# CLSFramework/gym-soccer-2d-env

Measured on AMD Instinct MI355X. Metric: env-steps/sec at 65536 parallel reach_ball envs per MI355X, higher is better.
Workload: dtype f32

## Files before the change

gym-soccer-2d-env_amd/csrc/s2d_engine.hip:

```cpp
#include <hip/hip_runtime.h>

#include <cmath>
#include <cstdio>
#include <cstdlib>
#include <cstring>
#include <new>
#include <string>
#include <type_traits>

#include "s2d_device.h"

#include "s2d_kernels.h"

__global__ void s2d_tables_kernel(S2DHot p, const S2DRare* __restrict__ rp, S2DTables* __restrict__ t) {
  if (blockIdx.x == 0 && threadIdx.x == 0 && rp->tab_len > 0) tables_build(p, rp->recover_init, rp->tab_power, rp->tab_len, *t);
}
__global__ __launch_bounds__(kBlock) void s2d_init_kernel(S2DHot p, const S2DRare* __restrict__ rp,
                                                          float* __restrict__ S, int64_t stride, int64_t n) {
  int64_t i = (int64_t)blockIdx.x * kBlock + threadIdx.x;
  if (i >= n) return;
  S[F_STAMINA * stride + i] = p.stamina_max;
  S[F_RECOVERY * stride + i] = rp->recover_init;
  S[F_EFFORT * stride + i] = p.effort_init;
  S[F_CAPACITY * stride + i] = p.stamina_capacity;
// ... 341 lines not shown
    if (p.auto_reset) n_missing += __popcll(__ballot(active && done != 0));
    if (ro.obs) store_obs_tile(lds[wv], ob, lane, active, ro.obs + (row + wave_first) * S2D_OBS_DIM, valid);
  }
  if (active) {
    if (fast) {
      const int q = e.step_number;
      e.stamina = tb->stamina[q]; e.effort = tb->effort[q]; e.recovery = tb->recovery[q]; e.capacity = tb->capacity[q];
    }
    env_store(e, S, stride, i);
    if (use_k) kplane[i] = k0 + (uint32_t)n_steps;
    o.reward[i] = reward; o.done[i] = (uint8_t)done; o.result[i] = (uint8_t)res;
    o.action_dir[i] = dir; o.action_cmd[i] = (uint8_t)cmd;
  }
  store_obs_tile(lds[wv], ob, lane, active, o.obs + wave_first * S2D_OBS_DIM, valid);
  if (!active) { cnt1 = cnt2 = cnt3 = 0; }
#pragma unroll
  for (int off = 32; off > 0; off >>= 1) {
    cnt1 += __shfl_xor(cnt1, off); cnt2 += __shfl_xor(cnt2, off); cnt3 += __shfl_xor(cnt3, off);
  }
  unsigned long long* const srow = stats_row(o.stats, wave_first);
  stats_store(srow, lane, stats_load(srow, lane), wave_first == 0 ? (unsigned long long)n * (unsigned long long)n_steps : 0ull, cnt1, cnt2, cnt3);
}

#ifndef S2D_NPRIO_S
#define S2D_NPRIO_S 3
#endif
#ifndef S2D_NPRIO_A
#define S2D_NPRIO_A 2
#endif
#ifndef S2D_NPRIO_B
#define S2D_NPRIO_B 2
#endif
#ifndef S2D_NPRIO_P
#define S2D_NPRIO_P 1
#endif
#ifndef S2D_PRIO_S
#define S2D_PRIO_S 1
#endif
#ifndef S2D_PRIO_A
#define S2D_PRIO_A 2
#endif
#ifndef S2D_PRIO_B
#define S2D_PRIO_B 3
#endif

#ifdef S2D_STAMPS
#define WS_STAMP_DECL uint64_t st_busy = 0, st_t0 = __builtin_amdgcn_s_memtime(); const uint64_t st_begin = st_t0, st_rt0 = __builtin_amdgcn_s_memrealtime()
#define WS_BARRIER() do { st_busy += __builtin_amdgcn_s_memtime() - st_t0; __syncthreads(); st_t0 = __builtin_amdgcn_s_memtime(); } while (0)
#define WS_STAMP_STORE() do { if (lane == 0) { float* q_ = o.terminal_obs + (wave_first + 2 * role) * S2D_OBS_DIM; \
    q_[0] = (float)st_busy; q_[1] = (float)(__builtin_amdgcn_s_memtime() - st_begin); q_[2] = (float)(st_rt0 & 0xffffff); \
    q_[3] = (float)(__builtin_amdgcn_s_memrealtime() & 0xffffff); \
    q_[4] = __int_as_float((int)__builtin_amdgcn_s_getreg((31 << 11) | 4)); q_[5] = __int_as_float((int)__builtin_amdgcn_s_getreg((31 << 11) | 20)); } } while (0)
#else
#define WS_STAMP_DECL do {} while (0)
#define WS_BARRIER() __syncthreads()
#define WS_STAMP_STORE() do {} while (0)
#endif

template <int MODE, int NK, int REC = 0>
__global__ __launch_bounds__(kWsBlock, 4) void s2d_reach_rollout_ws_kernel(S2DHot p_sgpr, const S2DRare* __restrict__ rp,
                                                                        float* __restrict__ S, int64_t stride,
                                                                        int64_t n, int n_steps,
                                                                        const void* __restrict__ actions, int kind,
                                                                        RolloutOut ro, StepOut o) {
  constexpr bool NOISE = NK != S2D_NK_OFF;
  constexpr int kActWords = NOISE ? (int)WA_WORDS : (int)WA_NPM;
  __shared__ float act[3][kActWords][kWave];
  __shared__ float snap[2][WS_WORDS][kWave];
  __shared__ float slots[kSlots][SL_WORDS][kWave];
  __shared__ __attribute__((aligned(16))) float tile[2][kObsTile];
  __shared__ float4 act_lut[kWave];
  __shared__ float ep_lds[S2D_TAB_MAX];
  __shared__ float2 sc_lut[361];
  const int lane = threadIdx.x & (kWave - 1);
  const int role = __builtin_amdgcn_readfirstlane(threadIdx.x / kWave);
  const bool nt = REC == 2 || (REC == 0 && ro.nt != 0);
  const int64_t wave_first = (int64_t)blockIdx.x * kWave;
  const int64_t i = wave_first + lane;
  const bool active = i < n;
  int64_t rows = n - wave_first; rows = rows > kWave ? kWave : rows;
  const int valid = (int)rows * S2D_OBS_DIM;
  const int n_iter = n_steps + 3;

  if (role != 1 && p_sgpr.auto_reset) {
    const uint64_t gid = (((uint64_t)p_sgpr.gid_hi << 32) | p_sgpr.gid_lo) + (uint64_t)i;
    uint32_t ep0 = 0u;
    if (active) ep0 = reinterpret_cast<const uint32_t*>(S + F_EPISODE * stride)[i];
    const int k = role == 0 ? 0 : role - 1;
    slot_fill_coop<NK>(p_sgpr, rp, slots[k], lane, (uint32_t)gid, (uint32_t)(gid >> 32), ep0 + 1u + (uint32_t)k, active,
                          reinterpret_cast<uint32_t*>(&tile[0][0]) + role * kWave);
  }

  if (role == 0) {
    if constexpr (NOISE) __builtin_amdgcn_s_setprio(S2D_NPRIO_P);
    const S2DHot& p = p_sgpr;
    const bool use_k = uses_policy_step<MODE, NOISE>(kind);
    uint32_t* const kplane = reinterpret_cast<uint32_t*>(S + F_POLICY * stride);
    uint32_t gl = 0, gh = 0, k0 = 0;
    if (active) {
      if (use_k) k0 = kplane[i];
      uint64_t gid = (((uint64_t)p.gid_hi << 32) | p.gid_lo) + (uint64_t)i;
      gl = (uint32_t)gid; gh = (uint32_t)(gid >> 32);
    }
    U4 quad{0, 0, 0, 0}, squad{0, 0, 0, 0}, nblk{0, 0, 0, 0};
    float dir = 0.0f; int cmd = 0;
    int64_t row = 0;
    const bool lut = MODE == S2D_MODE_DISCRETE && kind == S2D_ACT_RANDOM && p.n_actions <= kWave;
    if (lut && lane < p.n_actions) {
      int c0; float pw, d0;
      action_map<MODE>(p, Action4{(float)lane, 0.0f, 0.0f, 0.0f}, 0.0f, c0, pw, d0);
      const CmdPrep c = cmd_prepare(p, c0, pw, d0);
      act_lut[lane] = make_float4(c.power, c.dir, c.dir_rate, d0);
    }
    __syncthreads();
    WS_STAMP_DECL;
    int wslot = 0;
    auto policy_step = [&](int t) {
      if (active) {
        const uint32_t k = k0 + (uint32_t)t;
        CmdPrep c;
        if (lut) {
          if (t == 0 || (k & 3u) == 0u) quad = policy_quad(p, gl, gh, k, S2D_ST_POLICY);
          const int a = (int)rnd_below(quad_word(quad, k), (uint32_t)p.n_actions);
          if (REC != 0 || ro.action) rec_store(static_cast<int32_t*>(ro.action) + row + i, (int32_t)a, nt);
          const float4 e4 = act_lut[a];
          c = CmdPrep{e4.x, e4.y, e4.z}; dir = e4.w; cmd = S2D_CMD_DASH;
        } else {
          c = decide<MODE>(p, actions, kind, row + i, gl, gh, k, t == 0 || (k & 3u) == 0u, quad, squad, ro.action, cmd, dir);
        }
        const int b = wslot;
        if (MODE == S2D_MODE_TURN4) act[b][WA_CMD][lane] = __int_as_float(cmd);
        act[b][WA_POWER][lane] = c.power;
        act[b][WA_DIR][lane] = c.dir; act[b][WA_RATE][lane] = c.dir_rate;
        if constexpr (NK == S2D_NK_SQUARE) {
          const NoiseIn nz = noise_prepare_square(p, gl, gh, k, S2D_ST_NOISE, cmd == S2D_CMD_TURN);
          act[b][WA_NPM][lane] = nz.pm; act[b][WA_NPS][lane] = nz.ps; act[b][WA_NPC][lane] = nz.pc;
          act[b][WA_NBM][lane] = nz.bm; act[b][WA_NBS][lane] = nz.bs; act[b][WA_NBC][lane] = nz.bc;
          if (MODE == S2D_MODE_TURN4) act[b][WA_NTU][lane] = nz.tu;
        } else if constexpr (NOISE) {
          const NoiseWords nw = noise_words(p, gl, gh, k, S2D_ST_NOISE, cmd == S2D_CMD_TURN, nblk, t == 0 || (k & 1u) == 0u);
          const float2 ps = sc_lut[noise_dir_index(nw.wp)], bs = sc_lut[noise_dir_index(nw.wb)];
          act[b][WA_NPM][lane] = noise_mag(nw.wp); act[b][WA_NPS][lane] = ps.x; act[b][WA_NPC][lane] = ps.y;
          act[b][WA_NBM][lane] = noise_mag(nw.wb); act[b][WA_NBS][lane] = bs.x; act[b][WA_NBC][lane] = bs.y;
          if (MODE == S2D_MODE_TURN4) act[b][WA_NTU][lane] = nw.tu;
        }
        row += n;
      }
      wslot = wslot == 2 ? 0 : wslot + 1;
    };
    for (int s = 0; s < n_iter; ++s) {
      if (s == 0 && n_steps > 0) policy_step(0);
      if (s + 1 < n_steps) policy_step(s + 1);
      WS_BARRIER();
    }
    WS_STAMP_STORE();
    if (active) {
      if (use_k) kplane[i] = k0 + (uint32_t)n_steps;
      o.action_dir[i] = dir; o.action_cmd[i] = (uint8_t)cmd;
    }
  } else if (role == 1) {
    if constexpr (NOISE) __builtin_amdgcn_s_setprio(S2D_NPRIO_S);
    else __builtin_amdgcn_s_setprio(S2D_PRIO_S);
    const S2DHot p = hot_in_vgprs(p_sgpr);
    Env e;
    uint32_t gl = 0, gh = 0;
    int nth = 0, j = 0;
    if (active) {
      env_load(e, S, stride, i);
      uint64_t gid = (((uint64_t)p.gid_hi << 32) | p.gid_lo) + (uint64_t)i;
      gl = (uint32_t)gid; gh = (uint32_t)(gid >> 32);
      asm volatile("" ::"v"(e.px), "v"(e.py), "v"(e.vx), "v"(e.vy), "v"(e.body), "v"(e.stamina), "v"(e.effort),
                   "v"(e.recovery), "v"(e.capacity), "v"(e.bx), "v"(e.by), "v"(e.bvx), "v"(e.bvy),
                   "v"(e.step_number), "v"(e.cycle), "v"(e.episode));
    }
    const S2DTables* const tb = tables_of(rp);
    const int tab_len = MODE != S2D_MODE_TURN4 ? rp->tab_len : 0;
    bool fast = false;
    if (tab_len > 0) {
      bool ok = true;
      if (active) {
        const int sn = e.step_number;
        ok = sn >= 0 && sn < tab_len;
        const int q = ok ? sn : 0;
        ok = ok && e.stamina == tb->stamina[q] && e.effort == tb->effort[q] && e.recovery == tb->recovery[q] &&
             e.capacity == tb->capacity[q] && e.body == rintf(e.body) && fabsf(e.body) <= 180.0f;
      }
      fast = __ballot(active && !ok) == 0ull;
      if (fast)
        for (int k = lane; k < tab_len; k += kWave) ep_lds[k] = tb->ep[k];
    }
    if (fast || NK == S2D_NK_LATTICE) {
      for (int k = lane; k <= 360; k += kWave) {
        float sn, cs;
        sincos_deg((float)(k - 180), sn, cs);
        sc_lut[k] = make_float2(sn, cs);
      }
    }
    const ResetStamina rst = reset_stamina(p, rp);
    __syncthreads();
    WS_STAMP_DECL;
    auto loop = [&](auto fast_tag) {
      constexpr bool FAST = decltype(fast_tag)::value;
      struct ActRegs { float cmd, power, dir, rate, npm, nps, npc, nbm, nbs, nbc, ntu; };
      ActRegs cur{}, nxt{};
      float ep_cur = 0.0f; float2 sc_cur = make_float2(0.0f, 0.0f);
      int rslot = 1;
      auto fetch = [&](int slot) {
        ActRegs r{};
        if (MODE == S2D_MODE_TURN4) r.cmd = act[slot][WA_CMD][lane];
        if (!FAST) r.power = act[slot][WA_POWER][lane];
        r.dir = act[slot][WA_DIR][lane]; r.rate = act[slot][WA_RATE][lane];
        if constexpr (NOISE) {
          r.npm = act[slot][WA_NPM][lane]; r.nps = act[slot][WA_NPS][lane]; r.npc = act[slot][WA_NPC][lane];
          r.nbm = act[slot][WA_NBM][lane]; r.nbs = act[slot][WA_NBS][lane]; r.nbc = act[slot][WA_NBC][lane];
          if (MODE == S2D_MODE_TURN4) r.ntu = act[slot][WA_NTU][lane];
        }
        return r;
      };
      auto lookups = [&]() {
        if constexpr (FAST) {
          ep_cur = ep_lds[e.step_number];
          sc_cur = sc_lut[(int)norm_deg(e.body + cur.dir) + 180];
        }
      };
      auto simulate_iteration = [&](int s, auto steady_tag) {
        constexpr bool STEADY = decltype(steady_tag)::value;
        if ((STEADY || (s >= 1 && s <= n_steps)) && active) {
          if (!STEADY && s == 1) { cur = fetch(0); lookups(); }
          const bool more = STEADY || s < n_steps;
          if (more) nxt = fetch(rslot);
          const int b = (s - 1) & 1;
          int cmd = S2D_CMD_DASH;
          if (MODE == S2D_MODE_TURN4) cmd = __float_as_int(cur.cmd);
          NoiseIn nz{0.0f, 0.0f, 0.0f, 0.0f, 0.0f, 0.0f, 0.0f};
          if constexpr (NOISE) {
            nz = NoiseIn{cur.npm, cur.nps, cur.npc, cur.nbm, cur.nbs, cur.nbc, 0.0f};
            if (MODE == S2D_MODE_TURN4) nz.tu = cur.ntu;
          }
          float d2;
          if constexpr (FAST) {
            e.step_number += 1;
            d2 = sim_cycle_dash_fast<NOISE>(p, rp, e, ep_cur, cur.rate, sc_cur.x, sc_cur.y, nz);
          } else {
            const CmdPrep c{cur.power, cur.dir, cur.rate};
            e.step_number += 1;
            d2 = sim_cycle<NOISE, true>(p, rp, e, cmd, c, nz);
          }
          int flags = judge_sq(p, e.px, e.py, d2, e.step_number);
          const bool took = flags && p.auto_reset;
          snap[b][WS_PX][lane] = e.px; snap[b][WS_PY][lane] = e.py; snap[b][WS_BODY][lane] = e.body;
          snap[b][WS_BX][lane] = e.bx; snap[b][WS_BY][lane] = e.by;
          snap[b][WS_BVX][lane] = e.bvx; snap[b][WS_BVY][lane] = e.bvy;
          snap[b][WS_FLAGS][lane] = __int_as_float(flags | (j << 8));
          if (took) {
            if (nth >= kSlots)
              slot_fill<NK>(p, rp, slots[j], lane, gl, gh, (uint32_t)e.episode + 1u);
            episode_begin(e, slot_take<kWave>(slots[j], lane, rst));
            nth += 1; j = (j + 1 == kSlots) ? 0 : j + 1;
          }
          if (more) { cur = nxt; lookups(); }
        }
        if (STEADY || (s >= 1 && s < n_steps)) rslot = rslot == 2 ? 0 : rslot + 1;
        WS_BARRIER();
      };
      int s = 0;
      for (; s < 2 && s < n_iter; ++s) simulate_iteration(s, std::false_type{});
      for (; s < n_steps; ++s) simulate_iteration(s, std::true_type{});
      for (; s < n_iter; ++s) simulate_iteration(s, std::false_type{});
    };
    if (fast) {
      loop(std::true_type{});
      if (active) {
        const int q = e.step_number;
        e.stamina = tb->stamina[q]; e.effort = tb->effort[q]; e.recovery = tb->recovery[q]; e.capacity = tb->capacity[q];
      }
    } else {
      loop(std::false_type{});
    }
    WS_STAMP_STORE();
    if (active) {
      S[F_PX * stride + i] = e.px; S[F_PY * stride + i] = e.py;
      S[F_VX * stride + i] = e.vx; S[F_VY * stride + i] = e.vy;
      S[F_BODY * stride + i] = e.body;
      S[F_STAMINA * stride + i] = e.stamina; S[F_EFFORT * stride + i] = e.effort;
      S[F_RECOVERY * stride + i] = e.recovery; S[F_CAPACITY * stride + i] = e.capacity;
      S[F_BX * stride + i] = e.bx; S[F_BY * stride + i] = e.by;
      S[F_BVX * stride + i] = e.bvx; S[F_BVY * stride + i] = e.bvy;
      S[F_STEP * stride + i] = __int_as_float(e.step_number);
      S[F_CYCLE * stride + i] = __int_as_float(e.cycle);
      S[F_EPISODE * stride + i] = __int_as_float(e.episode);
    }
  } else if (role == 2) {
    __builtin_amdgcn_s_setprio(NOISE ? S2D_NPRIO_A : S2D_PRIO_A);
    const S2DHot p = hot_in_vgprs(p_sgpr);
    const bool auto_reset = p_sgpr.auto_reset != 0;
    float prev_dist = 0.0f, prev_angle = 0.0f;
    if (active) {
      prev_dist = S[F_PREV_DIST * stride + i]; prev_angle = S[F_PREV_ANGLE * stride + i];
      asm volatile("" ::"v"(prev_dist), "v"(prev_angle));
    }
    float oa[S2D_OBS_DIM];
    float reward = 0.0f; int res = 0, done = 0;
    unsigned int cnt1 = 0, cnt2 = 0, cnt3 = 0;
    unsigned long long* const srow = stats_row(o.stats, wave_first);
    const unsigned long long sold = stats_load(srow, lane);
    float* const term_row = o.terminal_obs + i * S2D_OBS_DIM;
    int64_t row = 0;
    __syncthreads();
    WS_STAMP_DECL;
    auto agent_iteration = [&](int s, auto steady_tag) {
      constexpr bool STEADY = decltype(steady_tag)::value;
      if (STEADY || (s >= 2 && s < n_steps + 2)) {
        const int b = s & 1;
        res = 0;
        if (active) {
          float px = snap[b][WS_PX][lane], py = snap[b][WS_PY][lane], body = snap[b][WS_BODY][lane];
          float bx = snap[b][WS_BX][lane], by = snap[b][WS_BY][lane];
          const int fw = __float_as_int(snap[b][WS_FLAGS][lane]);
          const int flags = fw & 0xff;
          float dist = hypot2(bx - px, by - py);
          float rel = observe_player(p, px, py, body, bx, by, oa);
          reward = reward_of(prev_dist, prev_angle, dist, rel, flags, res);
          prev_dist = dist; prev_angle = rel;
          done = flags ? 1 : 0;
          if (flags && auto_reset) {
            const float (*sl)[kWave] = slots[fw >> 8];
#pragma unroll
            for (int k = 0; k < 4; ++k) term_row[k] = oa[k];
#pragma unroll
            for (int k = 0; k < 4; ++k) oa[k] = sl[SL_FIRST + k][lane];
            prev_dist = sl[SL_DIST][lane]; prev_angle = sl[SL_REL][lane];
          }
          if (REC != 0 || ro.reward) rec_store(ro.reward + row + i, reward, nt);
          if (REC != 0 || ro.done) rec_store(ro.done + row + i, (uint8_t)done, nt);
          if (REC != 0 || ro.result) rec_store(ro.result + row + i, (uint8_t)res, nt);
          cnt1 += res == S2D_RESULT_GOAL; cnt2 += res == S2D_RESULT_OUT; cnt3 += res == S2D_RESULT_TIMEOUT;
          if (REC != 0 || ro.obs) {
            float* t = &tile[b][lane * S2D_OBS_DIM];
            t[0] = oa[0]; t[1] = oa[1]; t[2] = oa[2]; t[3] = oa[3];
          }
        }
        row += n;
      }
      WS_BARRIER();
    };
    {
      int s = 0;
      for (; s < 3 && s < n_iter; ++s) agent_iteration(s, std::false_type{});
      for (; s < n_steps + 2; ++s) agent_iteration(s, std::true_type{});
      for (; s < n_iter; ++s) agent_iteration(s, std::false_type{});
    }
    WS_STAMP_STORE();
    if (active) {
      S[F_PREV_DIST * stride + i] = prev_dist; S[F_PREV_ANGLE * stride + i] = prev_angle;
      o.reward[i] = reward; o.done[i] = (uint8_t)done; o.result[i] = (uint8_t)res;
#pragma unroll
      for (int k = 0; k < 4; ++k) o.obs[i * S2D_OBS_DIM + k] = oa[k];
    }
    if (!active) { cnt1 = cnt2 = cnt3 = 0; }
#pragma unroll
    for (int off = 32; off > 0; off >>= 1) {
      cnt1 += __shfl_xor(cnt1, off); cnt2 += __shfl_xor(cnt2, off); cnt3 += __shfl_xor(cnt3, off);
    }
    stats_store(srow, lane, sold, wave_first == 0 ? (unsigned long long)n * (unsigned long long)n_steps : 0ull, cnt1, cnt2, cnt3);
  } else {
    if constexpr (NOISE) __builtin_amdgcn_s_setprio(S2D_NPRIO_B);
    else __builtin_amdgcn_s_setprio(S2D_PRIO_B);
    const S2DHot p = hot_in_vgprs(p_sgpr);
    const bool auto_reset = p_sgpr.auto_reset != 0;
    float ob6[S2D_OBS_DIM];
    float* const term_row = o.terminal_obs + i * S2D_OBS_DIM;
    const bool obs_all_vec = valid == kObsTile && ((n * S2D_OBS_DIM * 4) & 15) == 0 &&
                             (reinterpret_cast<uintptr_t>(ro.obs + wave_first * S2D_OBS_DIM) & 15u) == 0;
    __syncthreads();
    WS_STAMP_DECL;
    auto ball_iteration = [&](int s, auto steady_tag) {
      constexpr bool STEADY = decltype(steady_tag)::value;
      if ((STEADY || s >= 3) && (REC != 0 || ro.obs))
        tile_flush(tile[(s - 1) & 1], lane, ro.obs + ((int64_t)(s - 3) * n + wave_first) * S2D_OBS_DIM, valid, nt, obs_all_vec);
      if ((STEADY || (s >= 2 && s < n_steps + 2)) && active) {
        const int b = s & 1;
        float bx = snap[b][WS_BX][lane], by = snap[b][WS_BY][lane];
        float bvx = snap[b][WS_BVX][lane], bvy = snap[b][WS_BVY][lane];
        const int fw = __float_as_int(snap[b][WS_FLAGS][lane]);
        observe_ball(p, bx, by, bvx, bvy, ob6);
        if ((fw & 0xff) && auto_reset) {
          const float (*sl)[kWave] = slots[fw >> 8];
#pragma unroll
          for (int k = 4; k < S2D_OBS_DIM; ++k) term_row[k] = ob6[k];
#pragma unroll
          for (int k = 4; k < S2D_OBS_DIM; ++k) ob6[k] = sl[SL_FIRST + k][lane];
        }
        if (REC != 0 || ro.obs) {
          float* t = &tile[b][lane * S2D_OBS_DIM];
#pragma unroll
          for (int k = 4; k < S2D_OBS_DIM; ++k) t[k] = ob6[k];
        }
      }
      WS_BARRIER();
    };
    {
      int s = 0;
      for (; s < 3 && s < n_iter; ++s) ball_iteration(s, std::false_type{});
      for (; s < n_steps + 2; ++s) ball_iteration(s, std::true_type{});
      for (; s < n_iter; ++s) ball_iteration(s, std::false_type{});
    }
    WS_STAMP_STORE();
    if (active) {
#pragma unroll
      for (int k = 4; k < S2D_OBS_DIM; ++k) o.obs[i * S2D_OBS_DIM + k] = ob6[k];
    }
  }
}

__global__ __launch_bounds__(kBlock) void s2d_world_model_kernel(const float* __restrict__ S, int64_t stride,
                                                                 int64_t n, S2DWorldModel w) {
  int64_t i = (int64_t)blockIdx.x * kBlock + threadIdx.x;
  if (i >= n) return;
  float px = S[F_PX * stride + i], py = S[F_PY * stride + i], vx = S[F_VX * stride + i], vy = S[F_VY * stride + i];
  float bx = S[F_BX * stride + i], by = S[F_BY * stride + i], bvx = S[F_BVX * stride + i], bvy = S[F_BVY * stride + i];
  float dx = bx - px, dy = by - py;
  float dist = hypot2(dx, dy), ang = atan2_deg(dy, dx);
  if (w.ball_dist_from_self) w.ball_dist_from_self[i] = dist;
  if (w.ball_angle_from_self) w.ball_angle_from_self[i] = ang;
  if (w.ball_relative_x) w.ball_relative_x[i] = dx;
  if (w.ball_relative_y) w.ball_relative_y[i] = dy;
  if (w.ball_pos_dist) w.ball_pos_dist[i] = hypot2(bx, by);
  if (w.ball_pos_angle) w.ball_pos_angle[i] = atan2_deg(by, bx);
  if (w.ball_vel_dist) w.ball_vel_dist[i] = hypot2(bvx, bvy);
  if (w.ball_vel_angle) w.ball_vel_angle[i] = atan2_deg(bvy, bvx);
  if (w.self_pos_dist) w.self_pos_dist[i] = hypot2(px, py);
  if (w.self_pos_angle) w.self_pos_angle[i] = atan2_deg(py, px);
  if (w.self_vel_dist) w.self_vel_dist[i] = hypot2(vx, vy);
  if (w.self_vel_angle) w.self_vel_angle[i] = atan2_deg(vy, vx);
  if (w.self_dist_from_ball) w.self_dist_from_ball[i] = dist;
  if (w.self_angle_from_ball) w.self_angle_from_ball[i] = atan2_deg(-dy, -dx);
}

enum { SV_NONFINITE, SV_BODY, SV_STAMINA, SV_EFFORT_RECOVERY, SV_COUNTERS, SV_OBS, SV_WORDS = 8 };
__global__ __launch_bounds__(kBlock) void s2d_validate_kernel(S2DHot p, const float* __restrict__ S, int64_t stride, int64_t n,
                                                              const float* __restrict__ obs, unsigned int* __restrict__ out) {
  const int64_t i = (int64_t)blockIdx.x * kBlock + threadIdx.x;
  if (i >= n) return;
  Env e;
  env_load(e, S, stride, i);
  const float w[15] = {e.px, e.py, e.vx, e.vy, e.body, e.stamina, e.effort, e.recovery, e.capacity, e.bx, e.by, e.bvx, e.bvy,
                       e.prev_dist, e.prev_angle};
  bool finite = true;
#pragma unroll
  for (int k = 0; k < 15; ++k) finite = finite && isfinite(w[k]);
  bool obs_ok = true;
#pragma unroll
  for (int k = 0; k < S2D_OBS_DIM; ++k) obs_ok = obs_ok && isfinite(obs[i * S2D_OBS_DIM + k]);
  if (!finite) atomicAdd(&out[SV_NONFINITE], 1u);
  if (!(fabsf(e.body) <= 180.0f) || !(fabsf(e.prev_angle) <= 180.0f)) atomicAdd(&out[SV_BODY], 1u);
  if (!(e.stamina >= 0.0f && e.stamina <= p.stamina_max) || !(e.capacity >= 0.0f || p.stamina_capacity < 0.0f)) atomicAdd(&out[SV_STAMINA], 1u);
  if (!(e.effort >= p.effort_min && e.effort <= p.effort_init) || !(e.recovery >= p.recover_min && e.recovery <= p.recover_init))
    atomicAdd(&out[SV_EFFORT_RECOVERY], 1u);
  if (e.step_number < 0 || e.episode < 0 || !(e.prev_dist >= 0.0f)) atomicAdd(&out[SV_COUNTERS], 1u);
  if (!obs_ok) atomicAdd(&out[SV_OBS], 1u);
}

__global__ void s2d_debug_eval_kernel(int op, const float* __restrict__ in, float* __restrict__ out, int64_t n) {
  int64_t i = (int64_t)blockIdx.x * blockDim.x + threadIdx.x;
  if (op == 9) {
    __shared__ uint32_t scratch[256];
    const uint32_t* u = reinterpret_cast<const uint32_t*>(in) + 4 * i;
    S2DHot p{}; p.seed_lo = u[2]; p.seed_hi = 0x5EEDu; p.half_l = 52.5f; p.half_w = 34.0f;
    S2DRare r{}; r.change_ball_position = 1; r.change_ball_velocity = 1; r.travel_factor = __uint_as_float(u[3]);
    const int lane = threadIdx.x & 63;
    const ResetSample a = reset_sample_coop(p, r, (uint32_t)i, 7u, u[0], u[1] != 0u, lane, scratch + (threadIdx.x & ~63u));
    const ResetSample b = reset_sample(p, r, (uint32_t)i, 7u, u[0]);
    float* q = out + 14 * i;
    q[0] = a.px; q[1] = a.py; q[2] = a.body; q[3] = a.bx; q[4] = a.by; q[5] = a.bvx; q[6] = a.bvy;
    q[7] = b.px; q[8] = b.py; q[9] = b.body; q[10] = b.bx; q[11] = b.by; q[12] = b.bvx; q[13] = b.bvy;
    return;
  }
  if (i >= n) return;
  switch (op) {
    case 10: {
      const uint32_t* u = reinterpret_cast<const uint32_t*>(in) + 4 * i;
      S2DHot p{}; p.seed_lo = u[3]; p.seed_hi = 0u;
      const NoiseIn nz = noise_prepare(p, u[0], u[1], u[2], S2D_ST_NOISE, false);
      float* q = out + 6 * i;
      q[0] = nz.pm; q[1] = nz.ps; q[2] = nz.pc; q[3] = nz.bm; q[4] = nz.bs; q[5] = nz.bc;
      break;
    }
    case 11:
    case 12: {
// ... 663 lines not shown
```

gym-soccer-2d-env_amd/csrc/s2d_kernels.h:

```cpp
#pragma once
#include <hip/hip_runtime.h>

#include <type_traits>

#include "s2d_device.h"
#include "s2d_net.h"

#define S2D_API extern "C" __attribute__((visibility("default")))

#ifndef S2D_BLOCK
#define S2D_BLOCK 256
#endif
static constexpr int kBlock = S2D_BLOCK;
static constexpr int kWavesPerBlock = kBlock / kWave;
static constexpr int kObsTile = kWave * S2D_OBS_DIM;
static constexpr int64_t kWsMaxEnvs = 524288;

struct StepOut {
  float* obs;
  float* reward;
  uint8_t* done;
  uint8_t* result;
  float* terminal_obs;
  float* action_dir;
  uint8_t* action_cmd;
  unsigned long long* stats;
  float* prep;
};

enum { PS_PX, PS_PY, PS_BODY, PS_BX, PS_BY, PS_BVX, PS_BVY, PS_WORDS };
S2D_DEV uint32_t* prep_tags(float* prep, int64_t stride) { return reinterpret_cast<uint32_t*>(prep + 2 * PS_WORDS * stride); }
static constexpr uint32_t kPrepTagMask = 0x3fffffffu;
S2D_DEV uint32_t prep_tag_of(uint32_t episode, const NextEpisode& q) {
  return (episode & kPrepTagMask) | ((uint32_t)__float_as_int(q.vx) & 0x80000000u) | (((uint32_t)__float_as_int(q.vy) & 0x80000000u) >> 1);
}

S2D_DEV void wave_lds_fence() {
  __builtin_amdgcn_fence(__ATOMIC_RELEASE, "wavefront");
  __builtin_amdgcn_wave_barrier();
  __builtin_amdgcn_fence(__ATOMIC_ACQUIRE, "wavefront");
}

S2D_DEV void tile_write(float* tile, const ObsOut& ob, int lane, bool active) {
  if (active) {
#pragma unroll
    for (int k = 0; k < S2D_OBS_DIM; ++k) tile[lane * S2D_OBS_DIM + k] = ob.o[k];
  }
}
typedef float v4f32_t __attribute__((ext_vector_type(4)));
S2D_DEV void rec_store16(float4* p, const float4& v, bool nt) {
  if (nt) {
    const v4f32_t w = {v.x, v.y, v.z, v.w};
    asm volatile("global_store_dwordx4 %0, %1, off nt" ::"v"(p), "v"(w) : "memory");
  } else {
    *p = v;
  }
}
template <typename T>
S2D_DEV void rec_store(T* p, T v, bool nt) {
  if (nt) __builtin_nontemporal_store(v, p); else *p = v;
}
S2D_DEV void tile_flush(const float* tile, int lane, float* __restrict__ dst, int valid, bool nt = false, bool all_vec = false) {
  const bool vec = all_vec || ((valid == kObsTile) && ((reinterpret_cast<uintptr_t>(dst) & 15u) == 0));
  if (vec) {
    const float4* t4 = reinterpret_cast<const float4*>(tile);
    float4* d4 = reinterpret_cast<float4*>(dst);
    rec_store16(d4 + lane, t4[lane], nt);
    rec_store16(d4 + kWave + lane, t4[kWave + lane], nt);
    if (lane < 32) rec_store16(d4 + 2 * kWave + lane, t4[2 * kWave + lane], nt);
  } else {
#pragma unroll
    for (int j = 0; j < S2D_OBS_DIM; ++j) {
      int idx = j * kWave + lane;
      if (idx < valid) dst[idx] = tile[idx];
    }
  }
}
S2D_DEV void store_obs_tile(float* tile, const ObsOut& ob, int lane, bool active, float* __restrict__ dst,
                            int valid) {
  tile_write(tile, ob, lane, active);
  wave_lds_fence();
  tile_flush(tile, lane, dst, valid);
  wave_lds_fence();
}

S2D_DEV unsigned long long* stats_row(unsigned long long* stats, int64_t wave_first) { return stats + (wave_first / kWave) * 8; }
S2D_DEV unsigned long long stats_load(const unsigned long long* row, int lane) { return lane < 4 ? row[lane] : 0ull; }
S2D_DEV void stats_store(unsigned long long* row, int lane, unsigned long long old, unsigned long long steps, unsigned int goal,
                         unsigned int out, unsigned int timeout) {
  const unsigned long long add = lane == 0 ? steps : lane == 1 ? goal : lane == 2 ? out : timeout;
  if (lane < 4 && add != 0ull) row[lane] = old + add;
}
S2D_DEV unsigned int wave_count(bool pred) { return (unsigned int)__popcll(__ballot(pred)); }

template <int MODE>
S2D_DEV Action4 load_action(const void* __restrict__ actions, int kind, int64_t idx) {
  Action4 a{0.0f, 0.0f, 0.0f, 0.0f};
  if (MODE == S2D_MODE_DISCRETE) {
    a.a0 = (kind == S2D_ACT_DISCRETE_I64) ? (float)static_cast<const long long*>(actions)[idx]
                                          : (float)static_cast<const int32_t*>(actions)[idx];
  } else if (MODE == S2D_MODE_CONT1) {
    a.a0 = static_cast<const float*>(actions)[idx];
  } else {
    float4 v = static_cast<const float4*>(actions)[idx];
    a.a0 = v.x; a.a1 = v.y; a.a2 = v.z; a.a3 = v.w;
  }
  return a;
}
template <int MODE>
S2D_DEV Action4 random_action(const S2DHot& p, uint32_t gid_lo, uint32_t gid_hi, uint32_t k, U4& quad, bool refresh) {
  Action4 a{0.0f, 0.0f, 0.0f, 0.0f};
  if (MODE == S2D_MODE_TURN4) {
    U4 w = s2d_draw(p, gid_lo, gid_hi, k, S2D_ST_POLICY, 1);
    a.a0 = rnd_u01(w.x) * 2.0f - 1.0f; a.a1 = rnd_u01(w.y) * 2.0f - 1.0f;
    a.a2 = rnd_u01(w.z) * 2.0f - 1.0f; a.a3 = rnd_u01(w.w) * 2.0f - 1.0f;
  } else {
    if (refresh) quad = policy_quad(p, gid_lo, gid_hi, k, S2D_ST_POLICY);
    uint32_t w = quad_word(quad, k);
    if (MODE == S2D_MODE_DISCRETE) a.a0 = (float)rnd_below(w, (uint32_t)p.n_actions);
    else a.a0 = rnd_u01(w) * 2.0f - 1.0f;
  }
  return a;
}
template <int MODE, bool NOISE>
S2D_DEV bool uses_policy_step(int kind) { return kind == S2D_ACT_RANDOM || MODE == S2D_MODE_TURN4 || NOISE; }

template <int MODE>
S2D_DEV void store_rollout_action(void* __restrict__ dst, int64_t idx, const Action4& a) {
  if (MODE == S2D_MODE_DISCRETE) static_cast<int32_t*>(dst)[idx] = (int32_t)a.a0;
  else if (MODE == S2D_MODE_CONT1) static_cast<float*>(dst)[idx] = a.a0;
  else static_cast<float4*>(dst)[idx] = make_float4(a.a0, a.a1, a.a2, a.a3);
}

template <int MODE>
S2D_DEV CmdPrep decide(const S2DHot& p, const void* __restrict__ actions, int kind, int64_t idx, uint32_t gid_lo,
                       uint32_t gid_hi, uint32_t k, bool refresh, U4& quad, U4& squad, void* __restrict__ action_out,
                       int& cmd, float& dir) {
  if (kind == S2D_ACT_COMMAND) {
    const float4 v = static_cast<const float4*>(actions)[idx];
    cmd = command_code(v.x); dir = v.z;
    return cmd_prepare(p, cmd, v.y, v.z);
  }
  Action4 a = (kind == S2D_ACT_RANDOM) ? random_action<MODE>(p, gid_lo, gid_hi, k, quad, refresh)
                                       : load_action<MODE>(actions, kind, idx);
  if (action_out) store_rollout_action<MODE>(action_out, idx, a);
  float u = 0.0f;
  if (MODE == S2D_MODE_TURN4) {
    if (refresh) squad = policy_quad(p, gid_lo, gid_hi, k, S2D_ST_SELECT);
    u = rnd_u01(quad_word(squad, k));
  }
  float power;
  action_map<MODE>(p, a, u, cmd, power, dir);
  return cmd_prepare(p, cmd, power, dir);
}

template <int MODE>
S2D_DEV CmdPrep decode_action(const S2DHot& p, const Action4& a, uint32_t gl, uint32_t gh, uint32_t k, bool refresh, U4& squad,
                              int& cmd, float& dir) {
// ... 173 lines not shown
```

Baseline: 105.8 billion.

## Specialize warp-specialized loops and use SGPR-based row stores to cut per-step overhead

Hoists one shared VGPR copy of the hot params for all roles. Splits the policy, agent and ball loops into compile-time variants (LUT vs. not, full wave vs. partial, vectorized obs flush vs. not), and adds a wave-uniform quiet check that skips the reward/reset branch when no lane finished. Record stores now use inline-asm global_store with a scalar row base and a per-lane 32-bit offset, avoiding 64-bit address math in each iteration. This adds code size and hand-written asm that depends on the row pointers being wave-uniform, plus an offline loop-stats script.

```diff
diff --git a/gym-soccer-2d-env_amd/csrc/s2d_engine.hip b/gym-soccer-2d-env_amd/csrc/s2d_engine.hip
--- a/gym-soccer-2d-env_amd/csrc/s2d_engine.hip
+++ b/gym-soccer-2d-env_amd/csrc/s2d_engine.hip
@@ -447,77 +447,84 @@
   const int valid = (int)rows * S2D_OBS_DIM;
   const int n_iter = n_steps + 3;
 
+  const S2DHot p_vgpr = hot_in_vgprs(p_sgpr);
+
   if (role != 1 && p_sgpr.auto_reset) {
     const uint64_t gid = (((uint64_t)p_sgpr.gid_hi << 32) | p_sgpr.gid_lo) + (uint64_t)i;
     uint32_t ep0 = 0u;
     if (active) ep0 = reinterpret_cast<const uint32_t*>(S + F_EPISODE * stride)[i];
     const int k = role == 0 ? 0 : role - 1;
-    slot_fill_coop<NK>(p_sgpr, rp, slots[k], lane, (uint32_t)gid, (uint32_t)(gid >> 32), ep0 + 1u + (uint32_t)k, active,
+    slot_fill_coop<NK>(p_vgpr, rp, slots[k], lane, (uint32_t)gid, (uint32_t)(gid >> 32), ep0 + 1u + (uint32_t)k, active,
                           reinterpret_cast<uint32_t*>(&tile[0][0]) + role * kWave);
   }
 
   if (role == 0) {
     if constexpr (NOISE) __builtin_amdgcn_s_setprio(S2D_NPRIO_P);
-    const S2DHot& p = p_sgpr;
     const bool use_k = uses_policy_step<MODE, NOISE>(kind);
     uint32_t* const kplane = reinterpret_cast<uint32_t*>(S + F_POLICY * stride);
     uint32_t gl = 0, gh = 0, k0 = 0;
     if (active) {
       if (use_k) k0 = kplane[i];
-      uint64_t gid = (((uint64_t)p.gid_hi << 32) | p.gid_lo) + (uint64_t)i;
+      uint64_t gid = (((uint64_t)p_sgpr.gid_hi << 32) | p_sgpr.gid_lo) + (uint64_t)i;
       gl = (uint32_t)gid; gh = (uint32_t)(gid >> 32);
     }
-    U4 quad{0, 0, 0, 0}, squad{0, 0, 0, 0}, nblk{0, 0, 0, 0};
     float dir = 0.0f; int cmd = 0;
-    int64_t row = 0;
-    const bool lut = MODE == S2D_MODE_DISCRETE && kind == S2D_ACT_RANDOM && p.n_actions <= kWave;
-    if (lut && lane < p.n_actions) {
+    const bool lut = MODE == S2D_MODE_DISCRETE && kind == S2D_ACT_RANDOM && p_sgpr.n_actions <= kWave;
+    if (lut && lane < p_sgpr.n_actions) {
       int c0; float pw, d0;
-      action_map<MODE>(p, Action4{(float)lane, 0.0f, 0.0f, 0.0f}, 0.0f, c0, pw, d0);
-      const CmdPrep c = cmd_prepare(p, c0, pw, d0);
+      action_map<MODE>(p_vgpr, Action4{(float)lane, 0.0f, 0.0f, 0.0f}, 0.0f, c0, pw, d0);
+      const CmdPrep c = cmd_prepare(p_vgpr, c0, pw, d0);
       act_lut[lane] = make_float4(c.power, c.dir, c.dir_rate, d0);
     }
     __syncthreads();
     WS_STAMP_DECL;
-    int wslot = 0;
-    auto policy_step = [&](int t) {
-      if (active) {
-        const uint32_t k = k0 + (uint32_t)t;
-        CmdPrep c;
-        if (lut) {
-          if (t == 0 || (k & 3u) == 0u) quad = policy_quad(p, gl, gh, k, S2D_ST_POLICY);
-          const int a = (int)rnd_below(quad_word(quad, k), (uint32_t)p.n_actions);
-          if (REC != 0 || ro.action) rec_store(static_cast<int32_t*>(ro.action) + row + i, (int32_t)a, nt);
-          const float4 e4 = act_lut[a];
-          c = CmdPrep{e4.x, e4.y, e4.z}; dir = e4.w; cmd = S2D_CMD_DASH;
-        } else {
-          c = decide<MODE>(p, actions, kind, row + i, gl, gh, k, t == 0 || (k & 3u) == 0u, quad, squad, ro.action, cmd, dir);
-        }
-        const int b = wslot;
-        if (MODE == S2D_MODE_TURN4) act[b][WA_CMD][lane] = __int_as_float(cmd);
-        act[b][WA_POWER][lane] = c.power;
-        act[b][WA_DIR][lane] = c.dir; act[b][WA_RATE][lane] = c.dir_rate;
-        if constexpr (NK == S2D_NK_SQUARE) {
-          const NoiseIn nz = noise_prepare_square(p, gl, gh, k, S2D_ST_NOISE, cmd == S2D_CMD_TURN);
-          act[b][WA_NPM][lane] = nz.pm; act[b][WA_NPS][lane] = nz.ps; act[b][WA_NPC][lane] = nz.pc;
-          act[b][WA_NBM][lane] = nz.bm; act[b][WA_NBS][lane] = nz.bs; act[b][WA_NBC][lane] = nz.bc;
-          if (MODE == S2D_MODE_TURN4) act[b][WA_NTU][lane] = nz.tu;
-        } else if constexpr (NOISE) {
-          const NoiseWords nw = noise_words(p, gl, gh, k, S2D_ST_NOISE, cmd == S2D_CMD_TURN, nblk, t == 0 || (k & 1u) == 0u);
-          const float2 ps = sc_lut[noise_dir_index(nw.wp)], bs = sc_lut[noise_dir_index(nw.wb)];
-          act[b][WA_NPM][lane] = noise_mag(nw.wp); act[b][WA_NPS][lane] = ps.x; act[b][WA_NPC][lane] = ps.y;
-          act[b][WA_NBM][lane] = noise_mag(nw.wb); act[b][WA_NBS][lane] = bs.x; act[b][WA_NBC][lane] = bs.y;
-          if (MODE == S2D_MODE_TURN4) act[b][WA_NTU][lane] = nw.tu;
+    auto policy_loop = [&](auto lut_tag) {
+      constexpr bool LUT = decltype(lut_tag)::value;
+      const S2DHot& p = p_vgpr;
+      U4 quad{0, 0, 0, 0}, squad{0, 0, 0, 0}, nblk{0, 0, 0, 0};
+      const uint32_t n_act = (uint32_t)p.n_actions;
+      int64_t row = 0;
+      int wslot = 0;
+      auto policy_step = [&](int t) {
+        if (active) {
+          const uint32_t k = k0 + (uint32_t)t;
+          CmdPrep c;
+          if constexpr (LUT) {
+            if (t == 0 || (k & 3u) == 0u) quad = policy_quad(p, gl, gh, k, S2D_ST_POLICY);
+            const int a = (int)rnd_below(quad_word(quad, k), n_act);
+            if (REC != 0 || ro.action) rec_store_row32(static_cast<int32_t*>(ro.action) + (row + wave_first), (uint32_t)lane * 4u, (uint32_t)a, nt);
+            const float4 e4 = act_lut[a];
+            c = CmdPrep{e4.x, e4.y, e4.z}; dir = e4.w; cmd = S2D_CMD_DASH;
+          } else {
+            c = decide<MODE>(p, actions, kind, row + i, gl, gh, k, t == 0 || (k & 3u) == 0u, quad, squad, ro.action, cmd, dir);
+          }
+          const int b = wslot;
+          if (MODE == S2D_MODE_TURN4) act[b][WA_CMD][lane] = __int_as_float(cmd);
+          act[b][WA_POWER][lane] = c.power;
+          act[b][WA_DIR][lane] = c.dir; act[b][WA_RATE][lane] = c.dir_rate;
+          if constexpr (NK == S2D_NK_SQUARE) {
+            const NoiseIn nz = noise_prepare_square(p, gl, gh, k, S2D_ST_NOISE, cmd == S2D_CMD_TURN);
+            act[b][WA_NPM][lane] = nz.pm; act[b][WA_NPS][lane] = nz.ps; act[b][WA_NPC][lane] = nz.pc;
+            act[b][WA_NBM][lane] = nz.bm; act[b][WA_NBS][lane] = nz.bs; act[b][WA_NBC][lane] = nz.bc;
+            if (MODE == S2D_MODE_TURN4) act[b][WA_NTU][lane] = nz.tu;
+          } else if constexpr (NOISE) {
+            const NoiseWords nw = noise_words(p, gl, gh, k, S2D_ST_NOISE, cmd == S2D_CMD_TURN, nblk, t == 0 || (k & 1u) == 0u);
+            const float2 ps = sc_lut[noise_dir_index(nw.wp)], bs = sc_lut[noise_dir_index(nw.wb)];
+            act[b][WA_NPM][lane] = noise_mag(nw.wp); act[b][WA_NPS][lane] = ps.x; act[b][WA_NPC][lane] = ps.y;
+            act[b][WA_NBM][lane] = noise_mag(nw.wb); act[b][WA_NBS][lane] = bs.x; act[b][WA_NBC][lane] = bs.y;
+            if (MODE == S2D_MODE_TURN4) act[b][WA_NTU][lane] = nw.tu;
+          }
         }
         row += n;
-      }
-      wslot = wslot == 2 ? 0 : wslot + 1;
+        wslot = wslot == 2 ? 0 : wslot + 1;
+      };
+      if (n_steps > 0) policy_step(0);
+      int s = 0;
+      for (; s + 1 < n_steps; ++s) { policy_step(s + 1); WS_BARRIER(); }
+      for (; s < n_iter; ++s) WS_BARRIER();
     };
-    for (int s = 0; s < n_iter; ++s) {
-      if (s == 0 && n_steps > 0) policy_step(0);
-      if (s + 1 < n_steps) policy_step(s + 1);
-      WS_BARRIER();
-    }
+    if (lut) policy_loop(std::true_type{});
+    else policy_loop(std::false_type{});
     WS_STAMP_STORE();
     if (active) {
       if (use_k) kplane[i] = k0 + (uint32_t)n_steps;
@@ -526,7 +533,7 @@
   } else if (role == 1) {
     if constexpr (NOISE) __builtin_amdgcn_s_setprio(S2D_NPRIO_S);
     else __builtin_amdgcn_s_setprio(S2D_PRIO_S);
-    const S2DHot p = hot_in_vgprs(p_sgpr);
+    const S2DHot& p = p_vgpr;
     Env e;
     uint32_t gl = 0, gh = 0;
     int nth = 0, j = 0;
@@ -657,7 +664,7 @@
     }
   } else if (role == 2) {
     __builtin_amdgcn_s_setprio(NOISE ? S2D_NPRIO_A : S2D_PRIO_A);
-    const S2DHot p = hot_in_vgprs(p_sgpr);
+    const S2DHot& p = p_vgpr;
     const bool auto_reset = p_sgpr.auto_reset != 0;
     float prev_dist = 0.0f, prev_angle = 0.0f;
     if (active) {
@@ -670,36 +677,48 @@
     unsigned long long* const srow = stats_row(o.stats, wave_first);
     const unsigned long long sold = stats_load(srow, lane);
     float* const term_row = o.terminal_obs + i * S2D_OBS_DIM;
-    int64_t row = 0;
+    int64_t row = wave_first;
+    const uint32_t off4 = (uint32_t)lane * 4u, off1 = (uint32_t)lane;
     __syncthreads();
     WS_STAMP_DECL;
-    auto agent_iteration = [&](int s, auto steady_tag) {
+    auto agent_iteration = [&](int s, auto steady_tag, auto full_tag) {
       constexpr bool STEADY = decltype(steady_tag)::value;
+      const bool active = decltype(full_tag)::value || i < n;
       if (STEADY || (s >= 2 && s < n_steps + 2)) {
         const int b = s & 1;
         res = 0;
+        float px = 0.0f, py = 0.0f, body = 0.0f, bx = 0.0f, by = 0.0f;
+        int fw = 0;
         if (active) {
-          float px = snap[b][WS_PX][lane], py = snap[b][WS_PY][lane], body = snap[b][WS_BODY][lane];
-          float bx = snap[b][WS_BX][lane], by = snap[b][WS_BY][lane];
-          const int fw = __float_as_int(snap[b][WS_FLAGS][lane]);
-          const int flags = fw & 0xff;
+          px = snap[b][WS_PX][lane]; py = snap[b][WS_PY][lane]; body = snap[b][WS_BODY][lane];
+          bx = snap[b][WS_BX][lane]; by = snap[b][WS_BY][lane];
+          fw = __float_as_int(snap[b][WS_FLAGS][lane]);
+        }
+        const int flags = fw & 0xff;
+        const bool quiet = __ballot(flags != 0) == 0ull;
+        if (active) {
           float dist = hypot2(bx - px, by - py);
           float rel = observe_player(p, px, py, body, bx, by, oa);
-          reward = reward_of(prev_dist, prev_angle, dist, rel, flags, res);
-          prev_dist = dist; prev_angle = rel;
-          done = flags ? 1 : 0;
-          if (flags && auto_reset) {
-            const float (*sl)[kWave] = slots[fw >> 8];
-#pragma unroll
-            for (int k = 0; k < 4; ++k) term_row[k] = oa[k];
-#pragma unroll
-            for (int k = 0; k < 4; ++k) oa[k] = sl[SL_FIRST + k][lane];
-            prev_dist = sl[SL_DIST][lane]; prev_angle = sl[SL_REL][lane];
+          reward = reward_of(prev_dist, prev_angle, dist, rel, 0, res);
+          done = 0;
+          float next_dist = dist, next_angle = rel;
+          if (!quiet) {
+            reward = reward_of(prev_dist, prev_angle, dist, rel, flags, res);
+            done = flags ? 1 : 0;
+            cnt1 += res == S2D_RESULT_GOAL; cnt2 += res == S2D_RESULT_OUT; cnt3 += res == S2D_RESULT_TIMEOUT;
+            if (flags && auto_reset) {
+              const float (*sl)[kWave] = slots[fw >> 8];
+#pragma unroll
+              for (int k = 0; k < 4; ++k) term_row[k] = oa[k];
+#pragma unroll
+              for (int k = 0; k < 4; ++k) oa[k] = sl[SL_FIRST + k][lane];
+              next_dist = sl[SL_DIST][lane]; next_angle = sl[SL_REL][lane];
+            }
           }
-          if (REC != 0 || ro.reward) rec_store(ro.reward + row + i, reward, nt);
-          if (REC != 0 || ro.done) rec_store(ro.done + row + i, (uint8_t)done, nt);
-          if (REC != 0 || ro.result) rec_store(ro.result + row + i, (uint8_t)res, nt);
-          cnt1 += res == S2D_RESULT_GOAL; cnt2 += res == S2D_RESULT_OUT; cnt3 += res == S2D_RESULT_TIMEOUT;
+          prev_dist = next_dist; prev_angle = next_angle;
+          if (REC != 0 || ro.reward) rec_store_row32(ro.reward + row, off4, (uint32_t)__float_as_int(reward), nt);
+          if (REC != 0 || ro.done) rec_store_row8(ro.done + row, off1, (uint32_t)done, nt);
+          if (REC != 0 || ro.result) rec_store_row8(ro.result + row, off1, (uint32_t)res, nt);
           if (REC != 0 || ro.obs) {
             float* t = &tile[b][lane * S2D_OBS_DIM];
             t[0] = oa[0]; t[1] = oa[1]; t[2] = oa[2]; t[3] = oa[3];
@@ -709,12 +728,14 @@
       }
       WS_BARRIER();
     };
-    {
+    auto agent_loop = [&](auto full_tag) {
       int s = 0;
-      for (; s < 3 && s < n_iter; ++s) agent_iteration(s, std::false_type{});
-      for (; s < n_steps + 2; ++s) agent_iteration(s, std::true_type{});
-      for (; s < n_iter; ++s) agent_iteration(s, std::false_type{});
-    }
+      for (; s < 3 && s < n_iter; ++s) agent_iteration(s, std::false_type{}, full_tag);
+      for (; s < n_steps + 2; ++s) agent_iteration(s, std::true_type{}, full_tag);
+      for (; s < n_iter; ++s) agent_iteration(s, std::false_type{}, full_tag);
+    };
+    if (valid == kObsTile) agent_loop(std::true_type{});
+    else agent_loop(std::false_type{});
     WS_STAMP_STORE();
     if (active) {
       S[F_PREV_DIST * stride + i] = prev_dist; S[F_PREV_ANGLE * stride + i] = prev_angle;
@@ -731,7 +752,7 @@
   } else {
     if constexpr (NOISE) __builtin_amdgcn_s_setprio(S2D_NPRIO_B);
     else __builtin_amdgcn_s_setprio(S2D_PRIO_B);
-    const S2DHot p = hot_in_vgprs(p_sgpr);
+    const S2DHot& p = p_vgpr;
     const bool auto_reset = p_sgpr.auto_reset != 0;
     float ob6[S2D_OBS_DIM];
     float* const term_row = o.terminal_obs + i * S2D_OBS_DIM;
@@ -739,15 +760,26 @@
                              (reinterpret_cast<uintptr_t>(ro.obs + wave_first * S2D_OBS_DIM) & 15u) == 0;
     __syncthreads();
     WS_STAMP_DECL;
-    auto ball_iteration = [&](int s, auto steady_tag) {
+    int64_t orow = wave_first;
+    auto ball_iteration = [&](int s, auto steady_tag, auto vec_tag) {
       constexpr bool STEADY = decltype(steady_tag)::value;
-      if ((STEADY || s >= 3) && (REC != 0 || ro.obs))
-        tile_flush(tile[(s - 1) & 1], lane, ro.obs + ((int64_t)(s - 3) * n + wave_first) * S2D_OBS_DIM, valid, nt, obs_all_vec);
-      if ((STEADY || (s >= 2 && s < n_steps + 2)) && active) {
-        const int b = s & 1;
-        float bx = snap[b][WS_BX][lane], by = snap[b][WS_BY][lane];
-        float bvx = snap[b][WS_BVX][lane], bvy = snap[b][WS_BVY][lane];
-        const int fw = __float_as_int(snap[b][WS_FLAGS][lane]);
+      constexpr bool VEC = decltype(vec_tag)::value;
+      constexpr bool FULL = STEADY && VEC;
+      const bool act = FULL || active;
+      const int b = s & 1;
+      float bx = 0.0f, by = 0.0f, bvx = 0.0f, bvy = 0.0f;
+      int fw = 0;
+      if ((STEADY || (s >= 2 && s < n_steps + 2)) && act) {
+        bx = snap[b][WS_BX][lane]; by = snap[b][WS_BY][lane];
+        bvx = snap[b][WS_BVX][lane]; bvy = snap[b][WS_BVY][lane];
+        fw = __float_as_int(snap[b][WS_FLAGS][lane]);
+      }
+      if ((STEADY || s >= 3) && (REC != 0 || ro.obs)) {
+        if constexpr (STEADY && VEC) tile_flush_vec(tile[(s - 1) & 1], lane, ro.obs + orow * S2D_OBS_DIM, nt);
+        else tile_flush(tile[(s - 1) & 1], lane, ro.obs + orow * S2D_OBS_DIM, valid, nt, obs_all_vec);
+        orow += n;
+      }
+      if ((STEADY || (s >= 2 && s < n_steps + 2)) && act) {
         observe_ball(p, bx, by, bvx, bvy, ob6);
         if ((fw & 0xff) && auto_reset) {
           const float (*sl)[kWave] = slots[fw >> 8];
@@ -764,12 +796,14 @@
       }
       WS_BARRIER();
     };
-    {
+    auto ball_loop = [&](auto vec_tag) {
       int s = 0;
-      for (; s < 3 && s < n_iter; ++s) ball_iteration(s, std::false_type{});
-      for (; s < n_steps + 2; ++s) ball_iteration(s, std::true_type{});
-      for (; s < n_iter; ++s) ball_iteration(s, std::false_type{});
-    }
+      for (; s < 3 && s < n_iter; ++s) ball_iteration(s, std::false_type{}, vec_tag);
+      for (; s < n_steps + 2; ++s) ball_iteration(s, std::true_type{}, vec_tag);
+      for (; s < n_iter; ++s) ball_iteration(s, std::false_type{}, vec_tag);
+    };
+    if (obs_all_vec && (REC != 0 || ro.obs)) ball_loop(std::true_type{});
+    else ball_loop(std::false_type{});
     WS_STAMP_STORE();
     if (active) {
 #pragma unroll
diff --git a/gym-soccer-2d-env_amd/csrc/s2d_kernels.h b/gym-soccer-2d-env_amd/csrc/s2d_kernels.h
--- a/gym-soccer-2d-env_amd/csrc/s2d_kernels.h
+++ b/gym-soccer-2d-env_amd/csrc/s2d_kernels.h
@@ -74,6 +74,29 @@
       int idx = j * kWave + lane;
       if (idx < valid) dst[idx] = tile[idx];
     }
+  }
+}
+S2D_DEV void rec_store_row32(void* row, uint32_t off, uint32_t v, bool nt) {
+  if (nt) asm volatile("global_store_dword %0, %1, %2 nt" ::"v"(off), "v"(v), "s"(row));
+  else asm volatile("global_store_dword %0, %1, %2" ::"v"(off), "v"(v), "s"(row));
+}
+S2D_DEV void rec_store_row8(void* row, uint32_t off, uint32_t v, bool nt) {
+  if (nt) asm volatile("global_store_byte %0, %1, %2 nt" ::"v"(off), "v"(v), "s"(row));
+  else asm volatile("global_store_byte %0, %1, %2" ::"v"(off), "v"(v), "s"(row));
+}
+S2D_DEV void tile_flush_vec(const float* tile, int lane, float* dst, bool nt) {
+  const v4f32_t* t4 = reinterpret_cast<const v4f32_t*>(tile);
+  const v4f32_t a = t4[lane], b = t4[kWave + lane], c = t4[2 * kWave + (lane & 31)];
+  asm volatile("" ::"v"(a), "v"(b), "v"(c));
+  const uint32_t off = (uint32_t)lane * 16u;
+  if (nt) {
+    asm volatile("global_store_dwordx4 %0, %1, %2 nt" ::"v"(off), "v"(a), "s"(dst));
+    asm volatile("global_store_dwordx4 %0, %1, %2 offset:1024 nt" ::"v"(off), "v"(b), "s"(dst));
+    if (lane < 32) asm volatile("global_store_dwordx4 %0, %1, %2 offset:2048 nt" ::"v"(off), "v"(c), "s"(dst));
+  } else {
+    asm volatile("global_store_dwordx4 %0, %1, %2" ::"v"(off), "v"(a), "s"(dst));
+    asm volatile("global_store_dwordx4 %0, %1, %2 offset:1024" ::"v"(off), "v"(b), "s"(dst));
+    if (lane < 32) asm volatile("global_store_dwordx4 %0, %1, %2 offset:2048" ::"v"(off), "v"(c), "s"(dst));
   }
 }
 S2D_DEV void store_obs_tile(float* tile, const ObsOut& ob, int lane, bool active, float* __restrict__ dst,
diff --git a/profiles/experiments/ws_loop_stats.py b/profiles/experiments/ws_loop_stats.py
--- /dev/null
+++ b/profiles/experiments/ws_loop_stats.py
@@ -0,0 +1,215 @@
+#!/usr/bin/env python3
+import argparse
+import os
+import re
+import subprocess
+import sys
+import tempfile
+
+ROOT = os.path.dirname(os.path.dirname(os.path.dirname(os.path.abspath(__file__))))
+CSRC = os.path.join(ROOT, 'gym-soccer-2d-env_amd', 'csrc')
+FLAGS = ['-O3', '-std=c++17', '--offload-arch=gfx950', '-ffp-contract=off', '-fPIC', '-fvisibility=hidden']
+
+ap = argparse.ArgumentParser()
+ap.add_argument('--mode', type=int, default=0)
+ap.add_argument('--noise', type=int, default=0)
+ap.add_argument('--rec', type=int, default=2)
+ap.add_argument('--asm')
+ap.add_argument('--hipcc', default=os.environ.get('HIPCC', '/opt/rocm/bin/hipcc'))
+ap.add_argument('--blocks', action='store_true', help='also list the basic blocks of every loop with their counts')
+a = ap.parse_args()
+
+if a.asm:
+    text = open(a.asm).read()
+else:
+    with tempfile.TemporaryDirectory() as d:
+        out = os.path.join(d, 's2d_engine.s')
+        subprocess.run([a.hipcc] + FLAGS + ['--cuda-device-only', '-S', '-o', out, os.path.join(CSRC, 's2d_engine.hip')],
+                       check=True, stderr=subprocess.DEVNULL)
+        text = open(out).read()
+
+sym = re.compile(r'^(_Z\d+s2d_reach_rollout_ws_kernelILi%dELi%dELi%dEE\w*):' % (a.mode, a.noise, a.rec), re.M)
+m = sym.search(text)
+if not m:
+    sys.exit(f'no instantiation <{a.mode}, {a.noise}, {a.rec}> in the assembly')
+name = m.group(1)
+end = text.index('.Lfunc_end', m.end())
+body = text[m.end():end].splitlines()
+info = text[end:text.index('; COMPUTE_PGM_RSRC2:USER_SGPR', end)]
+meta = text[text.index('.amdhsa_kernel ' + name):]
+meta = meta[:meta.index('.end_amdhsa_kernel')]
+
+
+def field(pat, src, default='?'):
+    mm = re.search(pat, src)
+    return mm.group(1) if mm else default
+
+
+VALU64 = re.compile(r'v_(lshl_add_u64|add_co_u32|sub_co_u32|add_u64|lshlrev_b64|lshrrev_b64|ashrrev_i64)')
+
+
+def classify(op):
+    if op == 's_barrier':
+        return 'barrier'
+    if op in ('v_readlane_b32', 'v_writelane_b32', 'v_readfirstlane_b32'):
+        return 'lane'
+    if op.startswith('v_'):
+        return 'valu'
+    if op.startswith('ds_'):
+        return 'lds'
+    if op.startswith(('global_', 'buffer_', 'flat_', 'scratch_')):
+        return 'vmem'
+    if op.startswith(('s_load', 's_buffer_load')):
+        return 'smem'
+    if op.startswith(('s_cbranch', 's_branch')):
+        return 'branch'
+    if op.startswith('s_waitcnt'):
+        return 'wait'
+    if op.startswith('s_'):
+        return 'salu'
+    return 'other'
+
+
+def instrs(lines):
+    for ln in lines:
+        t = ln.strip().split()
+        if t and not t[0].endswith(':') and not t[0].startswith(('.', ';')):
+            yield t[0], ln
+
+
+def mix(lines):
+    c = dict(valu=0, salu=0, lds=0, vmem=0, smem=0, branch=0, wait=0, lane=0, valu64=0, barrier=0, other=0)
+    for op, ln in instrs(lines):
+        k = classify(op)
+        if k == 'lane':
+            c['valu'] += 1
+            if op != 'v_readfirstlane_b32':
+                c['lane'] += 1
+        else:
+            c[k] += 1
+        if k == 'valu' and VALU64.match(op):
+            c['valu64'] += 1
+    return c
+
+
+starts = {0}
+for i, ln in enumerate(body):
+    if re.match(r'^\.LBB[0-9_]+:', ln):
+        starts.add(i)
+    elif re.match(r'\s+s_(c?branch\w*|endpgm)\b', ln):
+        starts.add(i + 1)
+starts = sorted(x for x in starts if x < len(body))
+blocks = [(x, y) for x, y in zip(starts, starts[1:] + [len(body)])]
+at = {}
+for k, (x, y) in enumerate(blocks):
+    mm = re.match(r'^(\.LBB[0-9_]+):', body[x])
+    if mm:
+        at[mm.group(1)] = k
+succ = [[] for _ in blocks]
+for k, (x, y) in enumerate(blocks):
+    last = None
+    for op, ln in instrs(body[x:y]):
+        last = (op, ln)
+    fall = True
+    if last:
+        mm = re.match(r'\s+s_(c?branch\w*)\s+(\.LBB[0-9_]+)', last[1])
+        if mm:
+            succ[k].append(at[mm.group(2)])
+            fall = mm.group(1) != 'branch'
+        elif last[0] == 's_endpgm':
+            fall = False
+    if fall and k + 1 < len(blocks):
+        succ[k].append(k + 1)
+pred = [[] for _ in blocks]
+for k, ss in enumerate(succ):
+    for t in ss:
+        pred[t].append(k)
+index, low, onstack, comp, stk, cnt = {}, {}, set(), {}, [], [0]
+for root in range(len(blocks)):
+    if root in index:
+        continue
+    work = [(root, 0)]
+    while work:
+        k, ci = work.pop()
+        if ci == 0:
+            index[k] = low[k] = cnt[0]
+            cnt[0] += 1
+            stk.append(k)
+            onstack.add(k)
+        recurse = False
+        for j in range(ci, len(succ[k])):
+            t = succ[k][j]
+            if t not in index:
+                work.append((k, j + 1))
+                work.append((t, 0))
+                recurse = True
+                break
+            if t in onstack:
+                low[k] = min(low[k], index[t])
+        if recurse:
+            continue
+        if low[k] == index[k]:
+            members = set()
+            while True:
+                q = stk.pop()
+                onstack.discard(q)
+                members.add(q)
+                if q == k:
+                    break
+            for q in members:
+                comp[q] = members
+        if work:
+            parent = work[-1][0]
+            low[parent] = min(low[parent], low[k])
+natural = {}
+for k, (x, y) in enumerate(blocks):
+    if any(op == 's_barrier' for op, _ in instrs(body[x:y])):
+        m = comp[k]
+        if len(m) > 1 or k in succ[k]:
+            natural[min(m)] = m
+inner = sorted(natural)
+
+
+def loop_lines(h):
+    out = []
+    for k in sorted(natural[h]):
+        out.extend(body[blocks[k][0]:blocks[k][1]])
+    return out
+
+
+def tile_waits(lines):
+    seq = list(instrs(lines))
+    rd = [k for k, (op, _) in enumerate(seq) if op.startswith('ds_read_b128')]
+    if not rd:
+        return None
+    st = [k for k, (op, _) in enumerate(seq) if op.startswith('global_store_dwordx4') and k > rd[-1]]
+    if not st:
+        return None
+    return sum(1 for op, ln in seq[rd[0]:st[0]] if op == 's_waitcnt' and 'lgkmcnt' in ln)
+
+
+n_spill = sum(1 for ln in body if 'SGPR spill to VGPR lane' in ln)
+n_wl = sum(1 for op, _ in instrs(body) if op == 'v_writelane_b32')
+n_rl = sum(1 for op, _ in instrs(body) if op == 'v_readlane_b32')
+print(f'kernel  s2d_reach_rollout_ws_kernel<{a.mode}, {a.noise}, {a.rec}>')
+print('VGPRs %s  SGPRs %s  SGPR spill registers %d (v_writelane %d, v_readlane %d in the whole kernel)  private segment %s B  '
+      'scratch %s B  LDS %s B  occupancy %s' % (
+          field(r'; NumVgprs: (\d+)', info), field(r'; TotalNumSgprs: (\d+)', info), n_spill, n_wl, n_rl,
+          field(r'\.amdhsa_private_segment_fixed_size (\d+)', meta), field(r'; ScratchSize: (\d+)', info),
+          field(r'; LDSByteSize: (\d+)', info), field(r'; Occupancy: (\d+)', info)))
+print(f'{len(inner)} loops with an s_barrier (strongly connected components of the control-flow graph; lines count from the kernel label):')
+print(f'{"lines":>13} {"blks":>4} {"VALU":>5} {"SALU":>5} {"LDS":>4} {"VMEM":>5} {"SMEM":>5} {"br":>3} {"wait":>5} {"lane":>5} {"VALU64":>7} '
+      f'{"bar":>4} {"tile lgkm waits":>16}')
+for h in inner:
+    ll = loop_lines(h)
+    c = mix(ll)
+    tw = tile_waits(ll)
+    ks = sorted(natural[h])
+    print(f'{blocks[ks[0]][0] + 1:6d}-{blocks[ks[-1]][1]:<6d} {len(ks):4d} {c["valu"]:5d} {c["salu"]:5d} {c["lds"]:4d} {c["vmem"]:5d} {c["smem"]:5d} '
+          f'{c["branch"]:3d} {c["wait"]:5d} {c["lane"]:5d} {c["valu64"]:7d} {c["barrier"]:4d} {"-" if tw is None else tw:>16}')
+    if a.blocks:
+        for k in ks:
+            x, y = blocks[k]
+            b = mix(body[x:y])
+            print(f'        block {x + 1:6d}-{y:<6d} VALU {b["valu"]:4d} SALU {b["salu"]:4d} LDS {b["lds"]:3d} VMEM {b["vmem"]:3d} '
+                  f'br {b["branch"]:2d} lane {b["lane"]:3d} VALU64 {b["valu64"]:2d}')
```

Measured after the change: 95.40 billion. 9.8% lower.
